# google-deepmind/open_spiel

Measured on AMD Instinct MI355X. Metric: env-steps/sec (batched LegalActions+ApplyAction+status, connect_four), higher is better.
Workload: dtype u64; 1 GPU; connect_four fused LegalActions+ApplyAction+status, 2^20 states/GPU, seed 0x5EED; states_per_gpu=1048576, parallelism=1 independent shard(s), no collective

## Files before the change

open_spiel_amd/csrc/osg_playout.hip:

```cpp
#include <algorithm>

#include "osg_batch_internal.h"

namespace {

template <class G>
__global__ void __launch_bounds__(kBlock)
k_random_steps(typename G::Params p, typename G::word_t* base, int64_t n, uint64_t seed, int64_t index_offset,
               int steps, unsigned long long* partials) {
  __shared__ unsigned long long s_sum[2][kBlock / 64];
  unsigned long long applied = 0, episodes = 0;
  const int64_t stride = static_cast<int64_t>(gridDim.x) * kBlock;
  for (int64_t i = static_cast<int64_t>(blockIdx.x) * kBlock + threadIdx.x; i < n; i += stride) {
    typename G::State s = G::load(p, base, n, i);
    Rng rng(seed, static_cast<uint64_t>(index_offset + i), 0);
    for (int t = 0; t < steps; ++t) {
      if (G::terminal(p, s)) {
        s = G::initial(p);
        ++episodes;
      }
      auto m = G::legal(p, s);
      int a = sample_action<G>(p, s, m, G::current_player(p, s), rng);
      G::apply(p, s, a);
      ++applied;
    }
    G::store(p, base, n, i, s);
  }
  unsigned long long a = applied, e = episodes;
#pragma unroll
  for (int off = 32; off >= 1; off >>= 1) {
    a += __shfl_xor(a, off);
    e += __shfl_xor(e, off);
  }
  if ((threadIdx.x & 63) == 0) {
    s_sum[0][threadIdx.x >> 6] = a;
    s_sum[1][threadIdx.x >> 6] = e;
  }
  __syncthreads();
  if (threadIdx.x == 0) {
    unsigned long long ta = 0, te = 0;
    for (int w = 0; w < kBlock / 64; ++w) { ta += s_sum[0][w]; te += s_sum[1][w]; }
    const int slot = blockIdx.x & (kCounterSlots - 1);
    atomicAdd(&partials[2 * slot], ta);
    atomicAdd(&partials[2 * slot + 1], te);
  }
}
__global__ void __launch_bounds__(64) k_fold_counters(unsigned long long* partials, unsigned long long* counters) {
  const int lane = threadIdx.x;
  unsigned long long a = partials[2 * lane], e = partials[2 * lane + 1];
  partials[2 * lane] = 0;
  partials[2 * lane + 1] = 0;
#pragma unroll
  for (int off = 32; off >= 1; off >>= 1) {
    a += __shfl_xor(a, off);
    e += __shfl_xor(e, off);
  }
  if (lane == 0) {
    counters[0] += a;
    counters[1] += e;
  }
}

constexpr uint64_t kSynthSub = 0x53594E5448ULL;
constexpr int kSynthMaxAttempts = 1 << 14;
template <class G>
__global__ void __launch_bounds__(kBlock)
k_synth(typename G::Params p, typename G::word_t* base, int64_t n, uint64_t seed, int64_t index_offset, int depth_mod,
        uint8_t* actions, int32_t* depth_out) {
  const int64_t i = static_cast<int64_t>(blockIdx.x) * kBlock + threadIdx.x;
  if (i >= n) return;
  Rng rng(seed, static_cast<uint64_t>(index_offset + i), kSynthSub);
  int depth = static_cast<int>(rng.below(static_cast<uint32_t>(depth_mod)));
  typename G::State s = G::initial(p);
  int t = 0, attempt = 0;
  for (;;) {
    const bool term = G::terminal(p, s);
    if (t == depth || term) {
      if (!term) break;
      if (++attempt >= kSynthMaxAttempts) { s = G::initial(p); depth = 0; break; }
      s = G::initial(p);
      t = 0;
      continue;
    }
    const auto m = G::legal(p, s);
    G::apply(p, s, sample_action<G>(p, s, m, G::current_player(p, s), rng));
    ++t;
  }
  G::store(p, base, n, i, s);
  const auto m = G::legal(p, s);
  const int a = sample_action<G>(p, s, m, G::current_player(p, s), rng);
  if (actions) actions[i] = static_cast<uint8_t>(a);
  if (depth_out) depth_out[i] = depth;
}

template <class G>
__global__ void __launch_bounds__(kBlock)
k_rollout(typename G::Params p, const typename G::word_t* base, int64_t n, int num_players, uint64_t seed,
          int64_t index_offset, int n_rollouts, int group, double* sum_returns, int32_t* steps_out) {
  const int64_t total = n * group;
  const int64_t stride = static_cast<int64_t>(gridDim.x) * kBlock;
  int64_t item = static_cast<int64_t>(blockIdx.x) * kBlock + threadIdx.x;
  if (item >= total) return;
  int64_t root = item / group;
  int r = static_cast<int>(item - root * group);
  typename G::State s = G::load(p, base, n, root);
  Rng rng(seed, static_cast<uint64_t>(index_offset + root), static_cast<uint64_t>(r));
  double acc[kMaxPlayers];
#pragma unroll
  for (int q = 0; q < kMaxPlayers; ++q) acc[q] = 0.0;
  int plies = 0, ply = 0;
  for (;;) {
    if (G::terminal(p, s) || ply >= kMaxPlayoutPlies) {
      double ret[kMaxPlayers];
      G::returns(p, s, ret);
#pragma unroll
      for (int q = 0; q < kMaxPlayers; ++q)
        if (q < num_players) acc[q] += ret[q];
      r += group;
      if (r >= n_rollouts) {
#pragma unroll
        for (int q = 0; q < kMaxPlayers; ++q) {
          if (q < num_players) sum_returns[item * num_players + q] = acc[q];
          acc[q] = 0.0;
        }
        if (steps_out) steps_out[item] = plies;
        plies = 0;
        item += stride;
        if (item >= total) break;
        root = item / group;
        r = static_cast<int>(item - root * group);
      }
      s = G::load(p, base, n, root);
      rng = Rng(seed, static_cast<uint64_t>(index_offset + root), static_cast<uint64_t>(r));
      ply = 0;
      continue;
    }
    auto m = G::legal(p, s);
    int a = sample_action<G>(p, s, m, G::current_player(p, s), rng);
    G::apply(p, s, a);
    ++plies;
    ++ply;
  }
}

template <class G>
__global__ void __launch_bounds__(kBlock)
k_rollout_hexfill(typename G::Params p, const typename G::word_t* base, int64_t n, uint64_t seed, int64_t index_offset,
                  int n_rollouts, int group, double* sum_returns) {
  const int64_t total = n * group;
  const int64_t stride = static_cast<int64_t>(gridDim.x) * kBlock;
  for (int64_t item = static_cast<int64_t>(blockIdx.x) * kBlock + threadIdx.x; item < total; item += stride) {
    const int64_t root = item / group;
    const typename G::State s = G::load(p, base, n, root);
    double acc = 0.0;
    for (int r = static_cast<int>(item - root * group); r < n_rollouts; r += group) {
      if (G::terminal(p, s)) {
        acc += G::result(s) == 1 ? 1.0 : -1.0;
        continue;
      }
      Rng rng(seed, static_cast<uint64_t>(index_offset + root), static_cast<uint64_t>(r));
      acc += G::fill_playout_winner(p, s, rng) == 0 ? 1.0 : -1.0;
    }
    sum_returns[item * 2] = acc;
    sum_returns[item * 2 + 1] = -acc + 0.0;
  }
}

template <class G>
void launch_rollout_hexfill(const typename G::Params& p, const void* words, int64_t n, uint64_t seed, int64_t index_offset,
                            int n_rollouts, int group, double* d_part, unsigned blocks, hipStream_t st) {
  if constexpr (is_hex<G>::value)
    k_rollout_hexfill<G><<<dim3(blocks), dim3(kBlock), 0, st>>>(p, static_cast<const typename G::word_t*>(words), n, seed,
                                                              index_offset, n_rollouts, group, d_part);
}

__global__ void __launch_bounds__(kBlock)
k_rollout_fold(const double* __restrict__ part, const int32_t* __restrict__ part_steps, int64_t n, int num_players,
               int group, double* __restrict__ sum_returns, int32_t* __restrict__ steps_out) {
  const int64_t k = static_cast<int64_t>(blockIdx.x) * kBlock + threadIdx.x;
  if (k >= n * num_players) return;
  const int64_t root = k / num_players;
  const int q = static_cast<int>(k - root * num_players);
  double v = 0.0;
  for (int j = 0; j < group; ++j) v += part[(root * group + j) * num_players + q];
  sum_returns[k] = v;
  if (steps_out && q == 0) {
    int32_t t = 0;
    for (int j = 0; j < group; ++j) t += part_steps[root * group + j];
    steps_out[root] = t;
  }
}

}

extern "C" {

int osg_random_steps(osg_batch* b, uint64_t seed, int64_t index_offset, int steps, unsigned long long* d_counters) {
  osg_ctx* ctx = b->ctx;
  unsigned long long* partials = ctx->d_illegal + 1;
  int64_t blocks = (b->n + kBlock - 1) / kBlock;
  constexpr int64_t kMaxBlocks = 4096;
  if (blocks > kMaxBlocks) blocks = kMaxBlocks;
  if (int rc = for_game(b->spec, [&](auto g, const auto& P) {
        using G = typename decltype(g)::type;
        k_random_steps<G><<<dim3(static_cast<unsigned>(blocks)), dim3(kBlock), 0, ctx->stream>>>(P,
            static_cast<typename G::word_t*>(b->words()), b->n, seed, index_offset,
            steps, partials);
        return OSG_OK;
      })) return rc;
  k_fold_counters<<<dim3(1), dim3(64), 0, ctx->stream>>>(partials, d_counters);
  OSG_HIP(hipGetLastError());
  return OSG_OK;
}

int osg_synth_batch(osg_batch* b, uint64_t seed, int64_t index_offset, int depth_mod, uint8_t* d_actions,
                    int32_t* d_depth) {
  if (!b) return set_error(OSG_ERR_INVALID, "osg_synth_batch: null batch");
  if (depth_mod < 1 || depth_mod > b->spec.desc.max_game_length)
    return set_error(OSG_ERR_INVALID, "osg_synth_batch: depth_mod must lie in [1, MaxGameLength()]");
  if (int rc = refuse_endless_playouts(b->spec, "osg_synth_batch")) return rc;
  if (d_actions && b->spec.desc.num_distinct_actions > 255)
    return set_error(OSG_ERR_UNSUPPORTED, "osg_synth_batch: d_actions holds one byte per action; pass NULL for games with more "
                                          "than 255 actions");
  osg_ctx* ctx = b->ctx;
  if (int rc = for_game(b->spec, [&](auto g, const auto& P) {
        using G = typename decltype(g)::type;
        k_synth<G><<<dim3(grid_for(b->n)), dim3(kBlock), 0, ctx->stream>>>(P,
            static_cast<typename G::word_t*>(b->words()), b->n, seed, index_offset, depth_mod,
            d_actions, d_depth);
        return OSG_OK;
      })) return rc;
  OSG_HIP(hipGetLastError());
  return OSG_OK;
}

int osg_rollout(const osg_batch* roots, uint64_t seed, int64_t index_offset, int n_rollouts, double* sum_returns,
                int32_t* steps, int on_host) {
  osg_ctx* ctx = roots->ctx;
  const int P_ = roots->spec.desc.num_players;
  const int64_t n = roots->n;
  if (n_rollouts <= 0) return set_error(OSG_ERR_INVALID, "n_rollouts must be positive");
  if (int rc = refuse_endless_playouts(roots->spec, "osg_rollout")) return rc;
  constexpr int kLanesLog2 = 19;
  int64_t group = ((int64_t{1} << kLanesLog2) + n - 1) / std::max<int64_t>(n, 1);
  if (group > n_rollouts) group = n_rollouts;
  if (group < 1) group = 1;
  const size_t ret_bytes = sizeof(double) * P_ * n, step_bytes = sizeof(int32_t) * n;
  const size_t off_steps = align_up(ret_bytes), off_part = on_host ? align_up(off_steps + step_bytes) : 0;
  const size_t part_bytes = group > 1 ? ret_bytes * group : 0, off_part_steps = align_up(off_part + part_bytes);
  const size_t scratch_bytes = group > 1 ? off_part_steps + step_bytes * group : (on_host ? off_steps + step_bytes : 0);
  char* scratch = nullptr;
  if (scratch_bytes) {
    void* ptr;
    int rc = osg_ctx_scratch(ctx, scratch_bytes, &ptr);
    if (rc) return rc;
    scratch = static_cast<char*>(ptr);
  }
  double* d_sum = on_host ? reinterpret_cast<double*>(scratch) : sum_returns;
  int32_t* d_steps = steps ? (on_host ? reinterpret_cast<int32_t*>(scratch + off_steps) : steps) : nullptr;
  double* d_part = group > 1 ? reinterpret_cast<double*>(scratch + off_part) : d_sum;
  int32_t* d_part_steps = d_steps ? (group > 1 ? reinterpret_cast<int32_t*>(scratch + off_part_steps) : d_steps) : nullptr;
  const int64_t total = n * group;
  int64_t blocks = (total + kBlock - 1) / kBlock;
  if (blocks > 2048) blocks = 2048;
  if (!steps && roots->spec.desc.game_kind == kHex) {
    if (int rc = for_game(roots->spec, [&](auto g, const auto& P) {
          using G = typename decltype(g)::type;
          launch_rollout_hexfill<G>(P, roots->words(), n, seed, index_offset, n_rollouts,
              static_cast<int>(group), d_part, static_cast<unsigned>(blocks), ctx->stream);
          return OSG_OK;
        })) return rc;
  } else {
  if (int rc = for_game(roots->spec, [&](auto g, const auto& P) {
        using G = typename decltype(g)::type;
        k_rollout<G><<<dim3(static_cast<unsigned>(blocks)), dim3(kBlock), 0, ctx->stream>>>(P,
            static_cast<const typename G::word_t*>(roots->words()), n, P_, seed,
            index_offset, n_rollouts, static_cast<int>(group), d_part,
            d_part_steps);
        return OSG_OK;
      })) return rc;
  }
  if (group > 1)
    k_rollout_fold<<<dim3(grid_for(n * P_)), dim3(kBlock), 0, ctx->stream>>>(d_part, d_part_steps, n, P_,
                                                                             static_cast<int>(group), d_sum, d_steps);
  OSG_HIP(hipGetLastError());
  if (on_host) {
    OSG_HIP(hipMemcpyAsync(sum_returns, d_sum, ret_bytes, hipMemcpyDeviceToHost, ctx->stream));
    if (steps) OSG_HIP(hipMemcpyAsync(steps, d_steps, step_bytes, hipMemcpyDeviceToHost, ctx->stream));
    OSG_HIP(hipStreamSynchronize(ctx->stream));
  }
  return OSG_OK;
}

}
```

Before: 255.2 billion env-steps/s.

## Add specialized connect-four random-step kernel with split 32-bit bitboards and LUT

Adds a dedicated kernel for standard connect_four that unpacks each state into mover/opponent 32-bit halves, runs branchless steps with terminal reset folded in, and picks the k-th open column through a shared-memory lookup table. It replaces the generic templated terminal/legal/sample/apply chain, aiming to cut 64-bit arithmetic, branching and per-step overhead. The counter reduction is moved into a shared helper. The cost is a separate code path that has to stay semantically identical to the generic one, including how the RNG draws are used.

Result: no change. 256.6 billion env-steps/s, median of 5 (+0.6%).

```diff
diff --git a/open_spiel_amd/csrc/osg_playout.hip b/open_spiel_amd/csrc/osg_playout.hip
--- a/open_spiel_amd/csrc/osg_playout.hip
+++ b/open_spiel_amd/csrc/osg_playout.hip
@@ -1,14 +1,36 @@
 #include <algorithm>
 
 #include "osg_batch_internal.h"
+#include "step/osg_c4_random_step.h"
 
 namespace {
+
+OSG_D void add_block_counters(unsigned long long applied, unsigned long long episodes, unsigned long long* partials) {
+  __shared__ unsigned long long s_sum[2][kBlock / 64];
+  unsigned long long a = applied, e = episodes;
+#pragma unroll
+  for (int off = 32; off >= 1; off >>= 1) {
+    a += __shfl_xor(a, off);
+    e += __shfl_xor(e, off);
+  }
+  if ((threadIdx.x & 63) == 0) {
+    s_sum[0][threadIdx.x >> 6] = a;
+    s_sum[1][threadIdx.x >> 6] = e;
+  }
+  __syncthreads();
+  if (threadIdx.x == 0) {
+    unsigned long long ta = 0, te = 0;
+    for (int w = 0; w < kBlock / 64; ++w) { ta += s_sum[0][w]; te += s_sum[1][w]; }
+    const int slot = blockIdx.x & (kCounterSlots - 1);
+    atomicAdd(&partials[2 * slot], ta);
+    atomicAdd(&partials[2 * slot + 1], te);
+  }
+}
 
 template <class G>
 __global__ void __launch_bounds__(kBlock)
 k_random_steps(typename G::Params p, typename G::word_t* base, int64_t n, uint64_t seed, int64_t index_offset,
                int steps, unsigned long long* partials) {
-  __shared__ unsigned long long s_sum[2][kBlock / 64];
   unsigned long long applied = 0, episodes = 0;
   const int64_t stride = static_cast<int64_t>(gridDim.x) * kBlock;
   for (int64_t i = static_cast<int64_t>(blockIdx.x) * kBlock + threadIdx.x; i < n; i += stride) {
@@ -26,24 +48,33 @@
     }
     G::store(p, base, n, i, s);
   }
-  unsigned long long a = applied, e = episodes;
-#pragma unroll
-  for (int off = 32; off >= 1; off >>= 1) {
-    a += __shfl_xor(a, off);
-    e += __shfl_xor(e, off);
-  }
-  if ((threadIdx.x & 63) == 0) {
-    s_sum[0][threadIdx.x >> 6] = a;
-    s_sum[1][threadIdx.x >> 6] = e;
+  add_block_counters(applied, episodes, partials);
+}
+
+__global__ void __launch_bounds__(kBlock)
+k_random_steps_c4std(uint64_t* base, int64_t n, uint64_t seed, int64_t index_offset, int steps,
+                     unsigned long long* partials) {
+  __shared__ uint8_t s_kth[7 * 128];
+  for (uint32_t e = threadIdx.x; e < 7u * 128u; e += kBlock) {
+    const uint32_t k = e >> 7, mask = e & 127u;
+    s_kth[e] = k < static_cast<uint32_t>(__builtin_popcount(mask)) ? static_cast<uint8_t>(c4_kth_open(mask, k)) : 0;
   }
   __syncthreads();
-  if (threadIdx.x == 0) {
-    unsigned long long ta = 0, te = 0;
-    for (int w = 0; w < kBlock / 64; ++w) { ta += s_sum[0][w]; te += s_sum[1][w]; }
-    const int slot = blockIdx.x & (kCounterSlots - 1);
-    atomicAdd(&partials[2 * slot], ta);
-    atomicAdd(&partials[2 * slot + 1], te);
-  }
+  const auto kth = [&](uint32_t mask, uint32_t k) -> uint32_t { return s_kth[(k << 7) + mask]; };
+  unsigned long long applied = 0, episodes = 0;
+  const int64_t stride = static_cast<int64_t>(gridDim.x) * kBlock;
+  for (int64_t i = static_cast<int64_t>(blockIdx.x) * kBlock + threadIdx.x; i < n; i += stride) {
+    C4Lane s = c4_lane_unpack(base[i], base[n + i]);
+    Rng rng(seed, static_cast<uint64_t>(index_offset + i), 0);
+    uint32_t resets = 0;
+#pragma unroll 2
+    for (int t = 0; t < steps; ++t) c4_random_step(s, rng, resets, kth);
+    base[i] = c4_lane_pack0(s);
+    base[n + i] = c4_lane_pack1(s);
+    applied += static_cast<unsigned long long>(steps > 0 ? steps : 0);
+    episodes += resets;
+  }
+  add_block_counters(applied, episodes, partials);
 }
 __global__ void __launch_bounds__(64) k_fold_counters(unsigned long long* partials, unsigned long long* counters) {
   const int lane = threadIdx.x;
@@ -201,7 +232,10 @@
   int64_t blocks = (b->n + kBlock - 1) / kBlock;
   constexpr int64_t kMaxBlocks = 4096;
   if (blocks > kMaxBlocks) blocks = kMaxBlocks;
-  if (int rc = for_game(b->spec, [&](auto g, const auto& P) {
+  if (b->spec.desc.game_kind == kC4 && b->spec.c4_std) {
+    k_random_steps_c4std<<<dim3(static_cast<unsigned>(blocks)), dim3(kBlock), 0, ctx->stream>>>(
+        static_cast<uint64_t*>(b->words()), b->n, seed, index_offset, steps, partials);
+  } else if (int rc = for_game(b->spec, [&](auto g, const auto& P) {
         using G = typename decltype(g)::type;
         k_random_steps<G><<<dim3(static_cast<unsigned>(blocks)), dim3(kBlock), 0, ctx->stream>>>(P,
             static_cast<typename G::word_t*>(b->words()), b->n, seed, index_offset,
diff --git a/open_spiel_amd/csrc/step/osg_c4_random_step.h b/open_spiel_amd/csrc/step/osg_c4_random_step.h
--- /dev/null
+++ b/open_spiel_amd/csrc/step/osg_c4_random_step.h
@@ -0,0 +1,84 @@
+#ifndef OSG_C4_RANDOM_STEP_H_
+#define OSG_C4_RANDOM_STEP_H_
+
+#include "osg_c4_step_split.h"
+
+namespace osg {
+
+struct C4Lane {
+  uint32_t mv_lo, mv_hi;
+  uint32_t ot_lo, ot_hi;
+  uint32_t flags;
+  uint32_t stones;
+};
+
+OSG_HD C4Lane c4_lane_unpack(uint64_t w0, uint64_t w1) {
+  const uint32_t x_lo = static_cast<uint32_t>(w0), x_hi = static_cast<uint32_t>(w0 >> 32) & 0x00FFFFFFu;
+  const uint32_t o_lo = static_cast<uint32_t>(w1), o_hi = static_cast<uint32_t>(w1 >> 32);
+  C4Lane s;
+  s.flags = static_cast<uint32_t>(w0 >> 56);
+  s.stones = static_cast<uint32_t>(__builtin_popcount(x_lo | o_lo) + __builtin_popcount(x_hi | o_hi));
+  const bool o_moves = (s.stones & 1u) != 0u;
+  s.mv_lo = o_moves ? o_lo : x_lo;
+  s.mv_hi = o_moves ? o_hi : x_hi;
+  s.ot_lo = o_moves ? x_lo : o_lo;
+  s.ot_hi = o_moves ? x_hi : o_hi;
+  return s;
+}
+OSG_HD uint64_t c4_lane_pack0(const C4Lane& s) {
+  const bool o_moves = (s.stones & 1u) != 0u;
+  const uint32_t lo = o_moves ? s.ot_lo : s.mv_lo, hi = o_moves ? s.ot_hi : s.mv_hi;
+  return (static_cast<uint64_t>(hi | (s.flags << 24)) << 32) | lo;
+}
+OSG_HD uint64_t c4_lane_pack1(const C4Lane& s) {
+  const bool o_moves = (s.stones & 1u) != 0u;
+  const uint32_t lo = o_moves ? s.mv_lo : s.ot_lo, hi = o_moves ? s.mv_hi : s.ot_hi;
+  return (static_cast<uint64_t>(hi) << 32) | lo;
+}
+
+OSG_HD uint32_t c4_kth_open(uint32_t mask, uint32_t k) {
+  uint32_t pos = 0;
+#pragma unroll
+  for (uint32_t width = 4; width >= 1; width >>= 1) {
+    const uint32_t low = mask & ((1u << width) - 1u);
+    const uint32_t c = static_cast<uint32_t>(__builtin_popcount(low));
+    const bool up = k >= c;
+    k -= up ? c : 0u;
+    mask = up ? mask >> width : low;
+    pos += up ? width : 0u;
+  }
+  return pos;
+}
+struct C4KthArith {
+  OSG_HD uint32_t operator()(uint32_t mask, uint32_t k) const { return c4_kth_open(mask, k); }
+};
+
+template <class Kth>
+OSG_HD uint32_t c4_random_step(C4Lane& s, Rng& rng, uint32_t& episodes, const Kth& kth) {
+  const bool over = (s.flags & 1u) != 0u;
+  episodes += s.flags & 1u;
+  const uint32_t mv_lo = over ? 0u : s.mv_lo, mv_hi = over ? 0u : s.mv_hi;
+  const uint32_t ot_lo = over ? 0u : s.ot_lo, ot_hi = over ? 0u : s.ot_hi;
+  const uint32_t stones = over ? 0u : s.stones;
+  const uint32_t all_lo = mv_lo | ot_lo, all_hi = mv_hi | ot_hi;
+  const uint32_t mask = c4_open_columns(all_lo, all_hi);
+  const uint32_t k = rng.below(static_cast<uint32_t>(__builtin_popcount(mask)));
+  const uint32_t a = kth(mask, k);
+  const uint32_t sh = a * 7u;
+  const uint32_t col = static_cast<uint32_t>(((static_cast<uint64_t>(all_hi) << 32) | all_lo) >> sh);
+  const uint64_t put = static_cast<uint64_t>((col + 1u) & 0x3Fu) << sh;
+  const uint32_t b_lo = mv_lo | static_cast<uint32_t>(put), b_hi = mv_hi | static_cast<uint32_t>(put >> 32);
+  const bool win = c4_has_four(b_lo, b_hi);
+  const uint32_t mover = stones & 1u;
+  s.stones = stones + 1u;
+  const bool done = win | (s.stones == 42u);
+  s.flags = done ? (((win ? mover : 2u) << 1) | 1u) : 0u;
+  s.mv_lo = ot_lo;
+  s.mv_hi = ot_hi;
+  s.ot_lo = b_lo;
+  s.ot_hi = b_hi;
+  return a;
+}
+
+}
+#endif
```
